# cyoq/onitama-alphazero

Hardware: AMD Instinct MI355X
Metric: MCTS node-expansions/sec/GPU @400 sims; self-play games/sec at 1/2/4/8 GPU (higher is better)
Workload: dtype fp32 (fp16x3 split)

## Files before the change

include/onitama_az.h:

```cpp
#ifndef ONITAMA_AZ_H
#define ONITAMA_AZ_H

#include <stddef.h>
#include <stdint.h>

#ifdef __cplusplus
extern "C" {
#endif

#define OAZ_ABI_VERSION 5

enum { OAZ_RED = 0, OAZ_BLUE = 1 };
enum { OAZ_PAWN = 0, OAZ_KING = 1 };
enum {
    OAZ_CAPTURE = 0,
    OAZ_RED_WIN = 1,
    OAZ_BLUE_WIN = 2,
    OAZ_IN_PROGRESS = 3
};
enum { OAZ_NUM_CARDS = 16, OAZ_MAX_MOVES = 40 };

enum {
    OAZ_OK = 0,
    OAZ_ERR_ARG = -1,
// ... 138 lines not shown
int oaz_set_search_time(oaz_engine* eng, int64_t search_time_ns);
int oaz_last_sims(oaz_engine* eng, int* sims);
int oaz_search_playouts(oaz_engine* eng, int* out, int G);
int oaz_load_weights(oaz_engine* eng, const float* blob, size_t n);

size_t oaz_weight_tensor_count(int blocks);
int oaz_weight_tensor_info(int blocks, size_t i, char* name, size_t name_cap, size_t* numel);
int oaz_weights_from_named(int blocks, const char* const* names, const float* const* data, const size_t* sizes,
                           size_t n, float* out, size_t out_n);
int oaz_load_weights_named(oaz_engine* eng, const char* const* names, const float* const* data,
                           const size_t* sizes, size_t n);
int oaz_ot_read(const char* path, float* out, size_t cap, size_t* n_out, int* blocks_out);
int oaz_load_ot(oaz_engine* eng, const char* path);
int oaz_ot_write(const char* path, const float* blob, size_t n, int blocks);
int oaz_checkpoint_path(const char* folder, int64_t iteration, int is_best, const char* stamp, char* out,
                        size_t cap);
int oaz_sync(oaz_engine* eng);
int oaz_set_timing(oaz_engine* eng, int enable);
int oaz_kernel_times_get(oaz_engine* eng, oaz_kernel_times* out);
int oaz_kernel_times_reset(oaz_engine* eng);

int oaz_nn_forward(oaz_engine* eng, const oaz_state* s, int B, float* policy, float* value);
int oaz_nn_fallbacks(oaz_engine* eng, uint64_t* tiles);

int oaz_search(oaz_engine* eng, const oaz_state* roots, int G, oaz_move* out_move,
               float* out_pi, float* out_root_value, oaz_search_stats* stats);
int oaz_tree_dump(oaz_engine* eng, int game, oaz_node* out, int cap, int* n_nodes);

int oaz_selfplay_reset(oaz_engine* eng);
int oaz_selfplay_step(oaz_engine* eng, int moves);
int oaz_selfplay_stats_get(oaz_engine* eng, oaz_selfplay_stats* out);
int oaz_samples_fetch(oaz_engine* eng, oaz_sample* out, size_t cap, size_t* n_out);
int oaz_samples_export_device(oaz_engine* eng, void* dev_dst, size_t cap_bytes, size_t* n_out);
int oaz_selfplay_run(oaz_engine* eng, int n_games, oaz_sample* out, size_t cap,
                     size_t* n_out, oaz_selfplay_stats* stats);

typedef struct oaz_comm oaz_comm;
typedef struct oaz_comm_id { char internal[128]; } oaz_comm_id;

int oaz_comm_unique_id(oaz_comm_id* out);
oaz_comm* oaz_comm_init(const oaz_comm_id* id, int rank, int world, int device);
void oaz_comm_destroy(oaz_comm* comm);
int oaz_allgather_samples(oaz_engine* eng, oaz_comm* comm, oaz_sample* dev_out, size_t cap, size_t* n_total,
                          uint64_t* counts_out);
int oaz_comm_allreduce_sum_f32(oaz_comm* comm, float* dev, size_t n, void* stream);
int oaz_comm_broadcast(oaz_comm* comm, void* dev, size_t bytes, int root, void* stream);
// ... 186 lines not shown
```

onitama-alphazero_amd/csrc/oaz_engine.cpp:

```cpp
#include <hip/hip_runtime.h>

#include <math.h>
#include <stddef.h>
#include <time.h>
#include <stdarg.h>
#include <stdio.h>
#include <stdlib.h>
#include <string.h>

#include <mutex>
#include <string>
#include <algorithm>
#include <vector>

#include "../../include/onitama_az.h"
#include "oaz_device.h"
#include "oaz_host.h"
#include "oaz_kernels.h"
#include "oaz_pack.h"
#include "oaz_weights_layout.h"

using namespace oaz;

static_assert(offsetof(oaz_config, search_time_ns) == 104 && sizeof(oaz_config) == 120, "oaz_config layout (ABI 4)");
// ... 658 lines not shown
extern "C" int oaz_nn_fallbacks(oaz_engine* e, uint64_t* tiles) {
    if (!e || !tiles) return oaz_set_err(OAZ_ERR_ARG, "nn_fallbacks: null");
    OAZ_ON_DEVICE(e->device);
    unsigned long long n = 0;
    HIP_TRY(hipMemcpyAsync(&n, e->nn_fallback, sizeof(n), hipMemcpyDeviceToHost, e->stream));
    HIP_TRY(hipStreamSynchronize(e->stream));
    *tiles = (uint64_t)n;
    return 0;
}

extern "C" int oaz_nn_forward(oaz_engine* e, const oaz_state* s, int B, float* policy, float* value) {
    if (!e || !s || B < 0) return oaz_set_err(OAZ_ERR_ARG, "nn_forward: bad arguments");
    if ((uint32_t)B > e->G) return oaz_set_err(OAZ_ERR_CAPACITY, "nn_forward: B=%d > games=%u", B, e->G);
    if (B == 0) return 0;
    OAZ_ON_DEVICE(e->device);
    HIP_TRY(hipMemcpyAsync(e->s_roots, s, (size_t)B * sizeof(oaz_state), hipMemcpyHostToDevice, e->stream));
    if (int rc = evaluate(e, e->s_roots, (uint32_t)B, e->s_rootp, e->s_rootv)) return rc;
    if (policy) HIP_TRY(hipMemcpyAsync(policy, e->s_rootp, (size_t)B * 50 * 4, hipMemcpyDeviceToHost, e->stream));
    if (value) HIP_TRY(hipMemcpyAsync(value, e->s_rootv, (size_t)B * 4, hipMemcpyDeviceToHost, e->stream));
    HIP_TRY(hipStreamSynchronize(e->stream));
    return 0;
}

static bool compact_leaves(const oaz_engine* e, uint32_t G) {
    return e->cfg.compact == 1 || (e->cfg.compact == 2 && G >= 12u * 16u * (uint32_t)e->cus);
}

enum SearchPath { PATH_LAT, PATH_GRP, PATH_STEPS };
static SearchPath search_path(const oaz_engine* e, uint32_t G, bool noise) {
    const bool one_launch = e->cfg.step_kernels == 0 && !compact_leaves(e, G) &&
                            (e->cfg.evaluator == OAZ_EVAL_HASH || e->cfg.precision == OAZ_FP32_SPLIT16) &&
                            tree_seg_kernels();
    if (!one_launch) return PATH_STEPS;
    if (!noise && G <= (uint32_t)e->cus) return PATH_LAT;
    return (G + 15) / 16 <= (uint32_t)e->cus ? PATH_GRP : PATH_STEPS;
}

static uint32_t noise_chunk_for(const oaz_engine* e) {
    if (search_path(e, e->G, true) != PATH_GRP) return kNoiseChunk;
    return std::max(kNoiseChunk, std::min((uint32_t)e->sims_cap, 512u));
}

constexpr uint32_t kAutoParts = 2048;
static int game_parts(const oaz_engine* e, uint32_t G) {
    int p = e->cfg.parts ? e->cfg.parts : (G >= kAutoParts ? 2 : 1);
    while (p > 1 && (uint32_t)(p - 1) * ((G + (uint32_t)p - 1) / (uint32_t)p) >= G) p /= 2;
// ... 475 lines not shown
```

onitama-alphazero_amd/csrc/oaz_nn.hip:

```cpp
#include <hip/hip_runtime.h>

#include <utility>

#include "oaz_device.h"
#include "oaz_kernels.h"

namespace oaz {

typedef float f32x4 __attribute__((ext_vector_type(4)));
typedef __bf16 bf16x8 __attribute__((ext_vector_type(8)));

namespace nn {
constexpr int kCh = 64;
constexpr int kSB = 16;
constexpr int kWaves = 8;
constexpr int kTPW = 13;
constexpr int kRS = 72;
constexpr int kScratch = 128;
constexpr int kLdsFloats = kSB * 25 * kRS + kWaves * kScratch;
}

struct TileSpan {
    int b0, end, cap;
};
__device__ __forceinline__ TileSpan tile_span(const TileMap& tm, int B) {
    if (!tm.bcnt) return TileSpan{(int)blockIdx.x * nn::kSB, B, B};
    const int b = (int)blockIdx.x % tm.nb, t = (int)blockIdx.x / tm.nb, base = b << kBucketShift;
    return TileSpan{base + t * nn::kSB, base + (int)tm.bcnt[b], tm.cap};
}

namespace x6 {
constexpr int kRowB = 384;
constexpr int kImageB = nn::kSB * 25 * kRowB;
constexpr int kLdsFloats = kImageB / 4 + nn::kWaves * nn::kScratch;
}

namespace h3 {
constexpr int kRowB = 128;
constexpr int kPlaneB = nn::kSB * 25 * kRowB;
constexpr int kImageB = 2 * kPlaneB;
constexpr int kLdsFloats = kImageB / 4 + nn::kWaves * nn::kScratch;
constexpr int kLutB = 256 * 16;
constexpr int kLutOff = kLdsFloats * 4;
}

__constant__ int8_t c_sq_order[25] = {0, 4, 20, 24, 1, 3, 21, 23, 6, 8, 12, 16, 18,
                                      2, 5, 10, 15, 9, 14, 19, 22, 7, 11, 13, 17};

__device__ __forceinline__ int nbr_index(int sq, int t) {
    const int r = sq / 5 + t / 3 - 1, c = sq % 5 + t % 3 - 1;
    return (r >= 0 && r < 5 && c >= 0 && c < 5) ? r * 5 + c : 25;
}

__device__ __forceinline__ int mover_info(const oaz_state st) {
    const int blue = st.to_move & 1;
    const int c0 = (blue ? st.cards[2] : st.cards[0]) & 15, c1 = (blue ? st.cards[3] : st.cards[1]) & 15;
    return c0 | (c1 << 4) | (blue << 8);
// ... 452 lines not shown
            B.nstep = -1;
            for (int i = 0; i < m; ++i) {
                B.j[i] = L.j[q + i];
                B.nb[i] = L.nb[q + i];
            }
            q += m;
            P.b[P.nbat++] = B;
        }
    }
    int next = -1;
    for (int k = P.nbat - 1; k >= 0; --k)
        if (P.b[k].first) {
            P.b[k].nstep = next;
            next = P.b[k].t * 2 + P.b[k].m;
        }
    return P;
}
template <int GRP, int KH>
struct ConvPlanOf {
    static constexpr ConvPlan P = conv_plan(GRP, KH);
};

struct X6Cfg {
    static constexpr int WAVES = 8, KH = OAZ_H3_KH, NS = 15, GRP0 = 3, GRP1 = 4;
};
template <int BF_, int DBG_ = 0>
struct H3Cfg {
    static constexpr int kSplit = BF_ ? kH1Split : kH3Split;
    static constexpr int WAVES = 8, KH = OAZ_H3_KH, NS = kSplit > 12 ? kSplit : 25 - kSplit, GRP0 = BF_ ? 9 : 7,
                         GRP1 = BF_ ? 10 : 8, BF = BF_, DBG = DBG_;
};

template <int GRP, int KH, int K, int N>
__device__ __forceinline__ void x6_load(bf16x8 (&a)[N], const char* img, const int (&ab)[2][3], int piece) {
    constexpr ConvBatch B = ConvPlanOf<GRP, KH>::P.b[K];
#pragma unroll
    for (int q = 0; q < N; ++q)
        if (q < B.n) {
            const int off = B.nb[q] * (nn::kSB * x6::kRowB) + piece * 128;
            a[q] = *reinterpret_cast<const bf16x8*>(img + ab[B.m][off >> 16] + (off & 0xffff));
        }
}

template <int GRP, int KH, int K, int NS, int N>
__device__ __forceinline__ void x6_mfma(f32x4 (&acc)[NS], const bf16x8 (&a)[N], const bf16x8& bv) {
    constexpr ConvBatch B = ConvPlanOf<GRP, KH>::P.b[K];
#pragma unroll
    for (int q = 0; q < N; ++q)
        if (q < B.n) acc[B.j[q]] = __builtin_amdgcn_mfma_f32_16x16x32_bf16(a[q], bv, acc[B.j[q]], 0, 0, 0);
}

struct FragW {
    __amdgpu_buffer_rsrc_t r;
    int voff;
};
__device__ __forceinline__ FragW frag_w(const float* p, size_t floats, int lane, int nt) {
    FragW w;
    w.r = __builtin_amdgcn_make_buffer_rsrc((void*)p, (short)0, (int)(floats * 4), 0x00020000);
    w.voff = (nt * 64 + lane) * 16;
    return w;
}
__device__ __forceinline__ bf16x8 x6_ldb(const FragW& w, int entry) {
    return __builtin_bit_cast(bf16x8, __builtin_amdgcn_raw_buffer_load_b128(w.r, w.voff, entry * 64 * 16, 0));
}

template <class C, int GRP, int K>
__device__ __forceinline__ void x6_step_b(const FragW& W, bf16x8 (&b)[3], bf16x8 (&bn)[3]) {
    constexpr ConvBatch B = ConvPlanOf<GRP, C::KH>::P.b[K];
    if constexpr (B.first && K > 0) {
#pragma unroll
        for (int pc = 0; pc < 3; ++pc) b[pc] = bn[pc];
    }
    if constexpr (B.first && B.nstep >= 0) {
#pragma unroll
        for (int pc = 0; pc < 3; ++pc) bn[pc] = x6_ldb(W, (B.nstep * 3 + pc) * 4);
    }
}

template <class C, int GRP, int K>
__device__ __forceinline__ void conv_x6_batch(f32x4 (&acc)[C::NS], const char* img, const FragW& W,
                                              bf16x8 (&b)[3], bf16x8 (&bn)[3], bf16x8 (&X)[C::KH],
                                              bf16x8 (&Y)[C::KH], const int (&ab)[2][3]) {
    constexpr int KH = C::KH, NS = C::NS;
    x6_step_b<C, GRP, K>(W, b, bn);
    x6_load<GRP, KH, K>(Y, img, ab, 0);
    x6_mfma<GRP, KH, K, NS>(acc, X, b[0]);
    x6_mfma<GRP, KH, K, NS>(acc, X, b[1]);
    x6_load<GRP, KH, K>(X, img, ab, 2);
    x6_mfma<GRP, KH, K, NS>(acc, Y, b[0]);
    x6_mfma<GRP, KH, K, NS>(acc, Y, b[1]);
    x6_mfma<GRP, KH, K, NS>(acc, Y, b[2]);
    if constexpr (K + 1 < ConvPlanOf<GRP, KH>::P.nbat) x6_load<GRP, KH, K + 1>(Y, img, ab, 1);
    x6_mfma<GRP, KH, K, NS>(acc, X, b[0]);
    __builtin_amdgcn_sched_barrier(0);
}

template <class C, int GRP, int... K>
__device__ __forceinline__ void conv_x6_run(f32x4 (&acc)[C::NS], const char* img, const FragW& W, const int (&lo)[2],
                                            std::integer_sequence<int, K...>) {
    int ab[2][3];
#pragma unroll
    for (int m = 0; m < 2; ++m)
#pragma unroll
        for (int sg = 0; sg < 3; ++sg) ab[m][sg] = lo[m] + sg * 65536;
    bf16x8 b[3], bn[3];
#pragma unroll
    for (int pc = 0; pc < 3; ++pc) b[pc] = x6_ldb(W, pc * 4);
    bf16x8 X[C::KH], Y[C::KH];
    x6_load<GRP, C::KH, 0>(X, img, ab, 1);
    ((K % 2 == 0 ? conv_x6_batch<C, GRP, K>(acc, img, W, b, bn, X, Y, ab)
                 : conv_x6_batch<C, GRP, K>(acc, img, W, b, bn, Y, X, ab)),
     ...);
}

template <class C, int GRP>
__device__ __forceinline__ void epilogue_x6_pack(const f32x4 (&acc)[C::NS], uint32_t (&pk)[C::NS][2][3],
                                                 const float* bias, f32x4 (&skip)[C::NS], int co, bool add,
                                                 bool keep) {
    const float bb = bias[co];
    const bool odd = co & 1;
    const float addf = add ? 1.0f : 0.0f;
    const uint32_t sel = odd ? 0x03020706u : 0x07060302u;
#pragma unroll
    for (int j = 0; j < grp_n(GRP); ++j) {
        float v[4];
#pragma unroll
        for (int r = 0; r < 4; ++r) {
            v[r] = __builtin_fmaf(skip[j][r], addf, acc[j][r] + bb);
            v[r] = v[r] > 0.0f ? v[r] : 0.0f;
            if (keep) skip[j][r] = v[r];
        }
#pragma unroll
        for (int k = 0; k < 2; ++k) {
            const float keep_ = odd ? v[2 * k + 1] : v[2 * k];
            const float send = odd ? v[2 * k] : v[2 * k + 1];
            const float got = __int_as_float(
                __builtin_amdgcn_update_dpp(0, __float_as_int(send), 0xB1, 0xF, 0xF, false));
            const uint32_t ka = __float_as_uint(keep_), ga = __float_as_uint(got);
            const float kr = keep_ - __uint_as_float(ka & 0xffff0000u), gr = got - __uint_as_float(ga & 0xffff0000u);
            const uint32_t kb = __float_as_uint(kr), gb = __float_as_uint(gr);
            const float kl = kr - __uint_as_float(kb & 0xffff0000u), gl = gr - __uint_as_float(gb & 0xffff0000u);
            pk[j][k][0] = __builtin_amdgcn_perm(ga, ka, sel);
            pk[j][k][1] = __builtin_amdgcn_perm(gb, kb, sel);
            pk[j][k][2] = __builtin_amdgcn_perm(__float_as_uint(gl), __float_as_uint(kl), sel);
        }
    }
}
template <class C, int GRP>
__device__ __forceinline__ void epilogue_x6_store(const uint32_t (&pk)[C::NS][2][3], char* img, const int (&eo)[2]) {
#pragma unroll
    for (int j = 0; j < grp_n(GRP); ++j)
#pragma unroll
        for (int k = 0; k < 2; ++k) {
            uint32_t* d = reinterpret_cast<uint32_t*>(img + grp_sq(GRP, j) * (nn::kSB * x6::kRowB) + eo[k]);
            d[0] = pk[j][k][0];
            d[32] = pk[j][k][1];
            d[64] = pk[j][k][2];
        }
}
template <class C, int GRP>
__device__ __forceinline__ void epilogue_x6(const f32x4 (&acc)[C::NS], char* img, const float* bias,
                                            f32x4 (&skip)[C::NS], const int (&eo)[2], int co, bool add, bool keep) {
    uint32_t pk[C::NS][2][3];
    epilogue_x6_pack<C, GRP>(acc, pk, bias, skip, co, add, keep);
    epilogue_x6_store<C, GRP>(pk, img, eo);
}

template <int GRP>
struct L1Regs {
    float w[9];
};
template <int GRP>
__device__ __forceinline__ void first_layer_x6_fetch(L1Regs<GRP>& R, const float* W, int lane, int nt) {
#pragma unroll
    for (int t = 0; t < 9; ++t) R.w[t] = W[(t * 4 + nt) * 64 + lane];
}
template <class C, int GRP>
__device__ __forceinline__ void first_layer_x6(f32x4 (&acc)[C::NS], const L1Regs<GRP>& R, const float* table,
                                               uint32_t bb, int cinfo, int lane, int nt) {
    const int kq = lane >> 4, co = nt * 16 + (lane & 15);
    constexpr int kBatch = 5;
    float tb[kBatch][5];
    auto fetch = [&](int j0) {
#pragma unroll
        for (int q = 0; q < kBatch; ++q)
            if (j0 + q < grp_n(GRP)) {
                const float* ts = table + (size_t)grp_sq(GRP, j0 + q) * 17 * nn::kCh + co;
#pragma unroll
// ... 17 lines not shown
        }
    const int c0 = cinfo & 15, c1 = (cinfo >> 4) & 15, blue = (cinfo >> 8) & 1;
    float a[5];
#pragma unroll
    for (int st = 0; st < 5; ++st) {
        const int k = 4 * st + kq;
        a[st] = k < 16 ? ((k == c0 || k == c1) ? 1.0f : 0.0f) : (k == 16 ? (float)blue : 0.0f);
    }
#pragma unroll
    for (int j0 = 0; j0 < grp_n(GRP); j0 += kBatch) {
#pragma unroll
        for (int st = 0; st < 5; ++st)
#pragma unroll
            for (int q = 0; q < kBatch; ++q)
                if (j0 + q < grp_n(GRP))
                    acc[j0 + q] = __builtin_amdgcn_mfma_f32_16x16x4f32(a[st], tb[q][st], acc[j0 + q], 0, 0, 0);
        if (j0 + kBatch < grp_n(GRP)) fetch(j0 + kBatch);
    }
}

template <class C, int GRP>
__device__ __forceinline__ void nn_x6_body(const oaz_state* __restrict__ states, const TileSpan sp,
                                           const float* __restrict__ blob, int blocks, float* __restrict__ policy,
                                           float* __restrict__ value, float* lds) {
    const int B = sp.end;
    constexpr int NS = C::NS;
    char* img = reinterpret_cast<char*>(lds);
    const int tid = threadIdx.x, wave = tid >> 6, lane = tid & 63;
    const int nt = wave & 3;
    const int b0 = sp.b0;
    int* pinfo = reinterpret_cast<int*>(lds + x6::kImageB / 4);
    const int co = nt * 16 + (lane & 15);
    const int i = lane & 15, kq = lane >> 4;
    int eo[2];
#pragma unroll
    for (int k = 0; k < 2; ++k) eo[k] = x6::elem_off(kq * 4 + 2 * k + (co & 1), co & ~1);
    const int lo[2] = {x6::chunk_off(i, 0, kq), x6::chunk_off(i, 0, 4 + kq)};

    f32x4 acc[NS];
    f32x4 skip[NS];
    {
        L1Regs<GRP> l1;
        first_layer_x6_fetch<GRP>(l1, blob + nnl::kL1B, lane, nt);
        const int b = min(b0 + i, sp.cap - 1);
        const uint32_t* w = reinterpret_cast<const uint32_t*>(&states[b]);
        const uint32_t bb = kq == 0 ? w[2] : kq == 1 ? w[0] : kq == 2 ? w[3] : w[1];
        if (tid < nn::kSB) pinfo[tid] = mover_info(states[b]);
        if (b0 >= B) return;
        __syncthreads();
#pragma unroll
        for (int j = 0; j < NS; ++j) acc[j] = skip[j] = f32x4{};
        first_layer_x6<C, GRP>(acc, l1, blob + nnl::kL1Table, bb, pinfo[i], lane, nt);
        epilogue_x6<C, GRP>(acc, img, blob + nnl::kL1Bias, skip, eo, co, false, true);
        __syncthreads();
    }
    const float* p = OAZ_NN_CONVS_AT(blob);
    for (int c = 0; c < 2 * blocks; ++c) {
#pragma unroll
        for (int j = 0; j < NS; ++j) acc[j] = f32x4{};
        conv_x6_run<C, GRP>(acc, img, frag_w(p, nnl::kConvW<OAZ_FP32_SPLIT>, lane, nt), lo,
                            std::make_integer_sequence<int, ConvPlanOf<GRP, C::KH>::P.nbat>{});
        p += nnl::kConvW<OAZ_FP32_SPLIT>;
        uint32_t pk[NS][2][3];
        epilogue_x6_pack<C, GRP>(acc, pk, p, skip, co, c & 1, c & 1);
        __syncthreads();
        epilogue_x6_store<C, GRP>(pk, img, eo);
        p += nnl::kConvTail<OAZ_FP32_SPLIT>;
        __syncthreads();
    }
    {
        const bf16x8* HB = reinterpret_cast<const bf16x8*>(p + nnl::kHeadB);
        bf16x8 hb[2][3];
#pragma unroll
        for (int m = 0; m < 2; ++m)
#pragma unroll
            for (int pc = 0; pc < 3; ++pc) hb[m][pc] = HB[(m * 3 + pc) * 64 + lane];
        constexpr int kSqPerWave = (25 + C::WAVES - 1) / C::WAVES;
        f32x4 hacc[kSqPerWave];
#pragma unroll
        for (int q = 0; q < kSqPerWave; ++q) {
            hacc[q] = f32x4{};
            const int sq = wave + q * C::WAVES;
            if (sq < 25) {
#pragma unroll
                for (int m = 0; m < 2; ++m) {
                    const char* a = img + sq * (nn::kSB * x6::kRowB) + lo[m];
                    const bf16x8 ah = *reinterpret_cast<const bf16x8*>(a);
                    const bf16x8 am = *reinterpret_cast<const bf16x8*>(a + 128);
                    const bf16x8 al = *reinterpret_cast<const bf16x8*>(a + 256);
                    hacc[q] = __builtin_amdgcn_mfma_f32_16x16x32_bf16(am, hb[m][0], hacc[q], 0, 0, 0);
                    hacc[q] = __builtin_amdgcn_mfma_f32_16x16x32_bf16(am, hb[m][1], hacc[q], 0, 0, 0);
                    hacc[q] = __builtin_amdgcn_mfma_f32_16x16x32_bf16(ah, hb[m][0], hacc[q], 0, 0, 0);
                    hacc[q] = __builtin_amdgcn_mfma_f32_16x16x32_bf16(ah, hb[m][1], hacc[q], 0, 0, 0);
                    hacc[q] = __builtin_amdgcn_mfma_f32_16x16x32_bf16(ah, hb[m][2], hacc[q], 0, 0, 0);
                    hacc[q] = __builtin_amdgcn_mfma_f32_16x16x32_bf16(al, hb[m][0], hacc[q], 0, 0, 0);
                }
            }
        }
        __syncthreads();
        float* feat = reinterpret_cast<float*>(img);
        const float hbias = i == 0 ? p[nnl::kBv] : i == 1 ? p[nnl::kBp] : p[nnl::kBp + 1];
#pragma unroll
        for (int q = 0; q < kSqPerWave; ++q) {
            const int sq = wave + q * C::WAVES;
            if (sq < 25 && i < 3)
#pragma unroll
                for (int r = 0; r < 4; ++r) {
                    const float v = hacc[q][r] + hbias;
                    feat[(kq * 4 + r) * 80 + i * 25 + sq] = v > 0.0f ? v : 0.0f;
                }
        }
        __syncthreads();
        constexpr int NP = nn::kSB / C::WAVES;
        const float* fq[NP];
        int bq[NP];
#pragma unroll
        for (int q = 0; q < NP; ++q) {
            fq[q] = feat + (wave + q * C::WAVES) * 80;
            bq[q] = b0 + wave + q * C::WAVES;
        }
        heads_mlp<NP>(fq, bq, p, lane, B, policy, value);
    }
}

template <class C>
__global__ void __launch_bounds__(64 * C::WAVES) k_nn_x6(const oaz_state* __restrict__ states, int B,
                                                        const float* __restrict__ blob, int blocks,
                                                        float* __restrict__ policy, float* __restrict__ value,
                                                        TileMap tm) {
    __shared__ __attribute__((aligned(16))) float lds[x6::kLdsFloats];
    const TileSpan sp = tile_span(tm, B);
    if ((threadIdx.x >> 8) == 0) {
        __builtin_amdgcn_s_setprio(1);
        nn_x6_body<C, C::GRP0>(states, sp, blob, blocks, policy, value, lds);
    } else {
        nn_x6_body<C, C::GRP1>(states, sp, blob, blocks, policy, value, lds);
// ... 457 lines not shown
        __syncthreads();
        stamp(4);
    };
    for (int c = 0; c < blocks; ++c) {
        conv_one(std::integral_constant<int, 0>{}, true);
        conv_one(std::integral_constant<int, 1>{}, c + 1 < blocks);
    }
    h3_heads<C>(p, img, lo, wave, lane, b0, B, policy, value);
    if constexpr (C::DBG == 2) {
        stamp(5);
        __syncthreads();
        float v = 0.0f;
#pragma unroll
        for (int k = 0; k < 8; ++k) v = lane == k ? (float)ph[k] : v;
        if (lane < 8 && b0 + nn::kSB <= B) policy[(size_t)b0 * 50 + wave * 8 + lane] = v;
    }
    if constexpr (C::BF) return false;
    return h3_overflowed(hmax);
}

template <class C>
struct H3Fallback {
    static constexpr bool kOn = !C::BF && C::DBG == 0;
    using X = X6Cfg;
    static constexpr int kBase = h3::kLdsFloats + h3::kLutB / 4;
    static constexpr int kLds = kOn && x6::kLdsFloats > kBase ? x6::kLdsFloats : kBase;
};

template <class X, int GRP>
__device__ __noinline__ void nn_h3_fallback(const oaz_state* __restrict__ states, const TileSpan sp,
                                            const float* __restrict__ xblob,
                                            int blocks, float* __restrict__ policy, float* __restrict__ value,
                                            float* lds) {
    nn_x6_body<X, GRP>(states, sp, xblob, blocks, policy, value, lds);
}

template <class C>
__global__ void __launch_bounds__(64 * C::WAVES) k_nn_h3(const oaz_state* __restrict__ states, int B,
                                                        const float* __restrict__ blob, int blocks,
                                                        float* __restrict__ policy, float* __restrict__ value,
                                                        const float* __restrict__ xblob,
                                                        unsigned long long* __restrict__ fallback, TileMap tm) {
    __shared__ __attribute__((aligned(16))) float lds[H3Fallback<C>::kLds];
    const uint64_t rt0 = C::DBG == 5 ? __builtin_amdgcn_s_memrealtime() : 0;
    const TileSpan sp = tile_span(tm, B);
    bool ovf;
    const bool g0 = (threadIdx.x >> 8) == 0;
    if (g0) {
        __builtin_amdgcn_s_setprio(1);
        ovf = nn_h3_body<C, C::GRP0>(states, sp, blob, blocks, policy, value, lds);
    } else {
        ovf = nn_h3_body<C, C::GRP1>(states, sp, blob, blocks, policy, value, lds);
    }
    if constexpr (H3Fallback<C>::kOn) {
        using X = typename H3Fallback<C>::X;
        if (__syncthreads_or(ovf)) {
            if (g0)
// ... 422 lines not shown
```

onitama-alphazero_amd/csrc/oaz_search_lat.hip:

```cpp
namespace oaz {

constexpr int kLatThreads = 512;

constexpr int kLatStateOff = h3s::kBytes;
constexpr int kLatVarsOff = kLatStateOff + 32;
constexpr int kLatPolOff = kLatVarsOff + 16;
constexpr int kLatStatOff = kLatPolOff + 52 * 4;
constexpr int kLatPathOff = kLatStatOff + GS_COUNT * 8;
constexpr int kLatPath = 2048;
constexpr int kLatSq = 2048;
constexpr int kLatLds = H3Fallback<H3Cfg<0>>::kLds * 4;
struct LatLayout {
    int root, sq, cache;
    uint32_t nsq, ncached;
};
__device__ __forceinline__ LatLayout lat_layout(uint32_t pathcap, bool path_lds, int sims, uint32_t cap) {
    LatLayout l;
    l.root = kLatPathOff + (path_lds ? (int)((pathcap * 4 + 15) & ~15u) : 0);
    l.sq = l.root + 32;
    l.nsq = (uint32_t)sims + 1 < (uint32_t)kLatSq ? (uint32_t)sims + 1 : (uint32_t)kLatSq;
    l.cache = (l.sq + (int)l.nsq * 8 + 31) & ~31;
    const uint32_t fit = (uint32_t)((kLatLds - l.cache) / (int)sizeof(oaz_node));
    l.ncached = fit < cap ? fit : cap;
    return l;
}

__device__ __noinline__ void lat_backup(const TreeView& t, const oaz_state* roots, const uint8_t* active,
                                        const float* policy, const float* value, uint32_t gs, float* sp,
                                        const NodesCached& na) {
    expand_backup_seg_body(t, roots, active, policy, value, gs, sp, na);
    __builtin_amdgcn_fence(__ATOMIC_RELEASE, "workgroup");
    __builtin_amdgcn_fence(__ATOMIC_ACQUIRE, "workgroup");
}
template <int DBG = 0>
// ... 115 lines not shown
        if (out) {
            *tg.n_nodes = *tl.n_nodes;
            *tg.leaf = *tl.leaf;
            *tg.depth = *tl.depth;
            *tg.leaf_state = *tl.leaf_state;
        } else {
            *tl.n_nodes = *tg.n_nodes;
            *tl.leaf = *tg.leaf;
            *tl.depth = *tg.depth;
            *tl.leaf_state = *tg.leaf_state;
        }
    }
}

template <int DBG = 0>
__global__ void __launch_bounds__(kLatThreads) k_search_lat(TreeView t, const oaz_state* __restrict__ roots,
                                                            const uint8_t* __restrict__ active, SearchParams prm,
                                                            int sims, int hash_eval, const float* __restrict__ blob,
                                                            int blocks, const float* __restrict__ xblob,
                                                            unsigned long long* __restrict__ fallback, float* policy,
                                                            float* value, const uint64_t* __restrict__ deadline,
                                                            uint32_t* __restrict__ sims_run) {
    using C = H3Cfg<0>;
    __shared__ __attribute__((aligned(16))) float lds[H3Fallback<C>::kLds];
    static_assert(kLatPathOff + kLatPath * 4 + 32 + kLatSq * 8 + 64 * (int)sizeof(oaz_node) <= kLatLds,
                  "k_search_lat LDS");
    const uint32_t g = blockIdx.x;
    if (g >= t.G || (active && active[g] != 1)) return;
    const int wave = (int)(threadIdx.x >> 6), lane = (int)(threadIdx.x & 63);
    const bool walker = wave == 4;
    char* const lb = reinterpret_cast<char*>(lds);
    TreeView tg = t;
    tg.nodes = t.nodes + (size_t)g * t.cap;
    tg.n_nodes = t.n_nodes + g;
    tg.path = t.path + (size_t)g * t.pathcap;
    tg.depth = t.depth + g;
    tg.leaf = t.leaf + g;
    tg.leaf_state = t.leaf_state + g;
    tg.stats = t.stats + (size_t)g * GS_COUNT;
    tg.need = nullptr;
    tg.slot = nullptr;
    tg.G = 1;
    const bool path_lds = t.pathcap <= (uint32_t)kLatPath;
    TreeView tl = tg;
    tl.leaf_state = reinterpret_cast<oaz_state*>(lb + kLatStateOff);
    tl.leaf = reinterpret_cast<uint32_t*>(lb + kLatVarsOff);
    tl.depth = tl.leaf + 1;
// ... 276 lines not shown
```

onitama-alphazero_amd/onitama_az/_abi.py:

```python
from __future__ import annotations

import ctypes as C
import os
from pathlib import Path

import numpy as np

LIB_NAME = "libonitama_az.so"
LIB_PATH = Path(__file__).resolve().parent / LIB_NAME

RED, BLUE = 0, 1
PAWN, KING = 0, 1
CAPTURE, RED_WIN, BLUE_WIN, IN_PROGRESS = 0, 1, 2, 3
EVAL_NN, EVAL_HASH = 0, 1
FP32, BF16, FP32_SPLIT, FP32_SPLIT16 = 0, 1, 2, 3
ERR_ARG = -1
ERR_RANGE = -7
ERR_CAPACITY = -4
ERR_COMM = -8
ABI_VERSION = 5
MAX_MOVES = 40


class OazError(RuntimeError):
# ... 278 lines not shown
    "oaz_encode": (C.c_int, [_VOIDP, C.c_int, _VOIDP]),
    "oaz_create": (_VOIDP, [_P(oaz_config), C.c_int]),
    "oaz_destroy": (None, [_VOIDP]),
    "oaz_get_config": (C.c_int, [_VOIDP, _P(oaz_config)]),
    "oaz_set_search_params": (C.c_int, [_VOIDP, C.c_int, C.c_double, C.c_int]),
    "oaz_set_search_time": (C.c_int, [_VOIDP, C.c_int64]),
    "oaz_last_sims": (C.c_int, [_VOIDP, _P(C.c_int)]),
    "oaz_search_playouts": (C.c_int, [_VOIDP, _VOIDP, C.c_int]),
    "oaz_load_weights": (C.c_int, [_VOIDP, _VOIDP, C.c_size_t]),
    "oaz_weight_tensor_count": (C.c_size_t, [C.c_int]),
    "oaz_weight_tensor_info": (C.c_int, [C.c_int, C.c_size_t, C.c_char_p, C.c_size_t, _P(C.c_size_t)]),
    "oaz_weights_from_named": (C.c_int, [C.c_int, _VOIDP, _VOIDP, _VOIDP, C.c_size_t, _VOIDP, C.c_size_t]),
    "oaz_load_weights_named": (C.c_int, [_VOIDP, _VOIDP, _VOIDP, _VOIDP, C.c_size_t]),
    "oaz_ot_read": (C.c_int, [C.c_char_p, _VOIDP, C.c_size_t, _P(C.c_size_t), _P(C.c_int)]),
    "oaz_load_ot": (C.c_int, [_VOIDP, C.c_char_p]),
    "oaz_ot_write": (C.c_int, [C.c_char_p, _VOIDP, C.c_size_t, C.c_int]),
    "oaz_checkpoint_path": (C.c_int, [C.c_char_p, C.c_int64, C.c_int, C.c_char_p, C.c_char_p, C.c_size_t]),
    "oaz_sync": (C.c_int, [_VOIDP]),
    "oaz_set_timing": (C.c_int, [_VOIDP, C.c_int]),
    "oaz_kernel_times_get": (C.c_int, [_VOIDP, _P(oaz_kernel_times)]),
    "oaz_kernel_times_reset": (C.c_int, [_VOIDP]),
    "oaz_nn_forward": (C.c_int, [_VOIDP, _VOIDP, C.c_int, _VOIDP, _VOIDP]),
    "oaz_nn_fallbacks": (C.c_int, [_VOIDP, _P(C.c_uint64)]),
    "oaz_search": (C.c_int, [_VOIDP, _VOIDP, C.c_int, _VOIDP, _VOIDP, _VOIDP, _P(oaz_search_stats)]),
    "oaz_tree_dump": (C.c_int, [_VOIDP, C.c_int, _VOIDP, C.c_int, _P(C.c_int)]),
    "oaz_selfplay_reset": (C.c_int, [_VOIDP]),
    "oaz_selfplay_step": (C.c_int, [_VOIDP, C.c_int]),
    "oaz_selfplay_stats_get": (C.c_int, [_VOIDP, _P(oaz_selfplay_stats)]),
    "oaz_samples_fetch": (C.c_int, [_VOIDP, _VOIDP, C.c_size_t, _P(C.c_size_t)]),
    "oaz_samples_export_device": (C.c_int, [_VOIDP, _VOIDP, C.c_size_t, _P(C.c_size_t)]),
    "oaz_selfplay_run": (C.c_int, [_VOIDP, C.c_int, _VOIDP, C.c_size_t, _P(C.c_size_t), _P(oaz_selfplay_stats)]),
    "oaz_comm_unique_id": (C.c_int, [_P(oaz_comm_id)]),
    "oaz_comm_init": (_VOIDP, [_P(oaz_comm_id), C.c_int, C.c_int, C.c_int]),
    "oaz_comm_destroy": (None, [_VOIDP]),
    "oaz_allgather_samples": (C.c_int, [_VOIDP, _VOIDP, _VOIDP, C.c_size_t, _P(C.c_size_t), _VOIDP]),
    "oaz_comm_allreduce_sum_f32": (C.c_int, [_VOIDP, _VOIDP, C.c_size_t, _VOIDP]),
    "oaz_comm_broadcast": (C.c_int, [_VOIDP, _VOIDP, C.c_size_t, C.c_int, _VOIDP]),
    "oaz_comm_sync": (C.c_int, [_VOIDP]),
    "oaz_comm_stats_get": (C.c_int, [_VOIDP, _P(oaz_comm_stats)]),
    "oaz_pure_mcts_config_default": (None, [_P(oaz_pure_mcts_config)]),
    "oaz_pure_mcts_tree_capacity": (C.c_size_t, [_P(oaz_pure_mcts_config)]),
    "oaz_pure_mcts_search": (C.c_int, [_VOIDP, C.c_int, _P(oaz_pure_mcts_config), _VOIDP, _VOIDP,
                                       _P(oaz_pure_mcts_stats), _VOIDP, C.c_size_t]),
    "oaz_pure_mcts_release_workspace": (C.c_int, [C.c_int]),
    "oaz_alphabeta_config_default": (None, [_P(oaz_alphabeta_config)]),
    "oaz_alphabeta_evaluate": (C.c_int, [_VOIDP, _VOIDP, C.c_int, _VOIDP]),
# ... 16 lines not shown
    "oaz_train_config_default": (None, [_P(oaz_train_config)]),
    "oaz_trainer_create": (_VOIDP, [_P(oaz_train_config), C.c_int]),
    "oaz_trainer_destroy": (None, [_VOIDP]),
    "oaz_trainer_set_stream": (C.c_int, [_VOIDP, _VOIDP]),
    "oaz_trainer_set_weights": (C.c_int, [_VOIDP, _VOIDP, C.c_size_t]),
    "oaz_trainer_get_weights": (C.c_int, [_VOIDP, _VOIDP, C.c_size_t]),
    "oaz_trainer_save_ot": (C.c_int, [_VOIDP, C.c_char_p]),
    "oaz_trainer_load_samples": (C.c_int, [_VOIDP, _VOIDP, C.c_size_t]),
    "oaz_trainer_bind_device_samples": (C.c_int, [_VOIDP, _VOIDP, C.c_size_t]),
    "oaz_trainer_set_batches": (C.c_int, [_VOIDP, _VOIDP, C.c_int, C.c_int]),
    "oaz_trainer_backward": (C.c_int, [_VOIDP, C.c_int]),
    "oaz_trainer_grads": (C.c_int, [_VOIDP, _P(C.c_void_p), _P(C.c_size_t)]),
    "oaz_trainer_get_grads": (C.c_int, [_VOIDP, _VOIDP, C.c_size_t]),
    "oaz_trainer_apply": (C.c_int, [_VOIDP, C.c_float]),
    "oaz_trainer_bn_stats_count": (C.c_size_t, [C.c_int]),
    "oaz_trainer_bn_stats_pack": (C.c_int, [_VOIDP, _VOIDP]),
    "oaz_trainer_bn_stats_unpack": (C.c_int, [_VOIDP, _VOIDP, C.c_float]),
    "oaz_trainer_train": (C.c_int, [_VOIDP, C.c_int, C.c_int]),
    "oaz_trainer_losses": (C.c_int, [_VOIDP, _P(C.c_double * 3)]),
    "oaz_trainer_sync": (C.c_int, [_VOIDP]),
}

EXPORTED_SYMBOLS = tuple(_PROTOS)

_lib = None


def load(path: str | os.PathLike | None = None) -> C.CDLL:
    global _lib
    if _lib is not None and path is None:
        return _lib
    p = Path(path) if path else Path(os.environ["OAZ_LIB"]) if os.environ.get("OAZ_LIB") else LIB_PATH
    if not p.exists():
        raise OazError(f"{p} not found: build it with `python -c 'import __graft_entry__ as g; g.build()'`")
    lib = C.CDLL(str(p), mode=C.RTLD_GLOBAL)
    for name, (res, args) in _PROTOS.items():
        fn = getattr(lib, name)
        fn.restype = res
        fn.argtypes = args
    if lib.oaz_abi_version() != ABI_VERSION:
        raise OazError("ABI version mismatch")
    if path is None:
        _lib = lib
    return lib


def check(rc: int) -> None:
    if rc < 0:
        msg = load().oaz_last_error()
        raise OazError(f"C ABI error {rc}: {msg.decode() if msg else ''}")


def ptr(a: np.ndarray) -> C.c_void_p:
    assert a.flags["C_CONTIGUOUS"]
    return C.c_void_p(a.ctypes.data)


def device_count() -> int:
    n = C.c_int(0)
    load().oaz_device_count(C.byref(n))
# ... 8 lines not shown
```

onitama-alphazero_amd/onitama_az/engine.py:

```python
from __future__ import annotations

import ctypes as C
from dataclasses import dataclass
from typing import Optional, Tuple

import numpy as np

from . import _abi


@dataclass
class SearchResult:
    moves: np.ndarray
    pi: np.ndarray
    root_value: Optional[np.ndarray]
    stats: _abi.oaz_search_stats


class Engine:

    def __init__(self, config: Optional[_abi.oaz_config] = None, device: int = 0, **overrides):
        lib = _abi.load()
        cfg = config if config is not None else _abi.default_config()
        for k, v in overrides.items():
# ... 42 lines not shown
        _abi.check(self._lib.oaz_set_search_time(self._h, int(round(float(seconds) * 1e9))))

    def last_sims(self) -> int:
        n = C.c_int(0)
        _abi.check(self._lib.oaz_last_sims(self._h, C.byref(n)))
        return int(n.value)

    def search_playouts(self, games: int) -> np.ndarray:
        out = np.zeros(int(games), dtype=np.int32)
        _abi.check(self._lib.oaz_search_playouts(self._h, _abi.ptr(out), int(games)))
        return out

    def sync(self) -> None:
        _abi.check(self._lib.oaz_sync(self._h))

    def nn_forward(self, states: np.ndarray) -> Tuple[np.ndarray, np.ndarray]:
        states = np.ascontiguousarray(states, dtype=_abi.STATE_DTYPE)
        B = len(states)
        pol = np.zeros((B, 2, 25), dtype=np.float32)
        val = np.zeros(B, dtype=np.float32)
        _abi.check(self._lib.oaz_nn_forward(self._h, _abi.ptr(states), B, _abi.ptr(pol), _abi.ptr(val)))
        return pol, val

    def nn_fallbacks(self) -> int:
        n = C.c_uint64(0)
        _abi.check(self._lib.oaz_nn_fallbacks(self._h, C.byref(n)))
        return int(n.value)

    def search(self, roots: np.ndarray, root_value: bool = False) -> SearchResult:
        roots = np.ascontiguousarray(roots, dtype=_abi.STATE_DTYPE)
        G = len(roots)
        moves = np.zeros(G, dtype=_abi.MOVE_DTYPE)
        pi = np.zeros((G, 2, 25), dtype=np.float32)
        rv = np.zeros(G, dtype=np.float32) if root_value else None
        st = _abi.oaz_search_stats()
        _abi.check(self._lib.oaz_search(self._h, _abi.ptr(roots), G, _abi.ptr(moves), _abi.ptr(pi),
                                        _abi.ptr(rv) if rv is not None else None, C.byref(st)))
        return SearchResult(moves, pi, rv, st)

    def tree(self, game: int) -> np.ndarray:
        n = C.c_int(0)
        _abi.check(self._lib.oaz_tree_dump(self._h, game, None, 0, C.byref(n)))
        out = np.zeros(n.value, dtype=_abi.NODE_DTYPE)
        _abi.check(self._lib.oaz_tree_dump(self._h, game, _abi.ptr(out), n.value, C.byref(n)))
        return out

# ... 40 lines not shown
```

Before: 51.60 million.

## Run the h3 fallback recompute in two half-tile passes within h3's LDS

The x6 fallback path inside the h3 network kernel now processes the 16-row tile in two 8-row passes, so its image fits in the h3 kernel's own LDS footprint. Previously the fallback's larger LDS need inflated the h3 kernel's and the latency search kernel's shared-memory allocation. The intent is to shrink per-block LDS and so raise occupancy for the common h3 path, at the cost of a slower fallback that now recomputes per half-tile. A tiled forward entry point is also added for testing the bucketed path.

```diff
diff --git a/include/onitama_az.h b/include/onitama_az.h
--- a/include/onitama_az.h
+++ b/include/onitama_az.h
@@ -184,6 +184,7 @@
 
 int oaz_nn_forward(oaz_engine* eng, const oaz_state* s, int B, float* policy, float* value);
 int oaz_nn_fallbacks(oaz_engine* eng, uint64_t* tiles);
+int oaz_nn_forward_tiled(oaz_engine* eng, const oaz_state* s, int B, int count, float* policy, float* value);
 
 int oaz_search(oaz_engine* eng, const oaz_state* roots, int G, oaz_move* out_move,
                float* out_pi, float* out_root_value, oaz_search_stats* stats);
diff --git a/onitama-alphazero_amd/csrc/oaz_engine.cpp b/onitama-alphazero_amd/csrc/oaz_engine.cpp
--- a/onitama-alphazero_amd/csrc/oaz_engine.cpp
+++ b/onitama-alphazero_amd/csrc/oaz_engine.cpp
@@ -704,6 +704,30 @@
     return 0;
 }
 
+extern "C" int oaz_nn_forward_tiled(oaz_engine* e, const oaz_state* s, int B, int count, float* policy, float* value) {
+    if (!e || !s || B < 0 || count > B) return oaz_set_err(OAZ_ERR_ARG, "nn_forward_tiled: bad arguments");
+    if ((uint32_t)B > e->G) return oaz_set_err(OAZ_ERR_CAPACITY, "nn_forward_tiled: B=%d > games=%u", B, e->G);
+    if (e->cfg.evaluator != OAZ_EVAL_NN) return oaz_set_err(OAZ_ERR_ARG, "nn_forward_tiled: the engine's evaluator is not the network");
+    if (count >= 0 && (uint32_t)B > kBucket) return oaz_set_err(OAZ_ERR_ARG, "nn_forward_tiled: one bucket holds %u rows", kBucket);
+    if (B == 0) return 0;
+    OAZ_ON_DEVICE(e->device);
+    const uint32_t cnt = count >= 0 ? (uint32_t)count : 0u;
+    HIP_TRY(hipMemcpyAsync(e->s_roots, s, (size_t)B * sizeof(oaz_state), hipMemcpyHostToDevice, e->stream));
+    const TileMap tm{e->bcnt, 1, B};
+    if (count >= 0) {
+        HIP_TRY(hipMemcpyAsync(e->bcnt, &cnt, sizeof(cnt), hipMemcpyHostToDevice, e->stream));
+        HIP_TRY(hipMemsetAsync(e->s_rootp, 0, (size_t)B * 50 * 4, e->stream));
+        HIP_TRY(hipMemsetAsync(e->s_rootv, 0, (size_t)B * 4, e->stream));
+    }
+    NNView w = nn_view(e, count >= 0 ? &tm : nullptr);
+    w.small_max = 0;
+    HIP_TRY(launch_nn_forward(w, e->s_roots, B, e->s_rootp, e->s_rootv, e->stream));
+    if (policy) HIP_TRY(hipMemcpyAsync(policy, e->s_rootp, (size_t)B * 50 * 4, hipMemcpyDeviceToHost, e->stream));
+    if (value) HIP_TRY(hipMemcpyAsync(value, e->s_rootv, (size_t)B * 4, hipMemcpyDeviceToHost, e->stream));
+    HIP_TRY(hipStreamSynchronize(e->stream));
+    return 0;
+}
+
 static bool compact_leaves(const oaz_engine* e, uint32_t G) {
     return e->cfg.compact == 1 || (e->cfg.compact == 2 && G >= 12u * 16u * (uint32_t)e->cus);
 }
diff --git a/onitama-alphazero_amd/csrc/oaz_nn.hip b/onitama-alphazero_amd/csrc/oaz_nn.hip
--- a/onitama-alphazero_amd/csrc/oaz_nn.hip
+++ b/onitama-alphazero_amd/csrc/oaz_nn.hip
@@ -33,6 +33,8 @@
 constexpr int kRowB = 384;
 constexpr int kImageB = nn::kSB * 25 * kRowB;
 constexpr int kLdsFloats = kImageB / 4 + nn::kWaves * nn::kScratch;
+constexpr int image_bytes(int rows) { return rows * 25 * kRowB; }
+constexpr int lds_floats(int rows) { return image_bytes(rows) / 4 + nn::kWaves * nn::kScratch; }
 }
 
 namespace h3 {
@@ -531,7 +533,10 @@
 };
 
 struct X6Cfg {
-    static constexpr int WAVES = 8, KH = OAZ_H3_KH, NS = 15, GRP0 = 3, GRP1 = 4;
+    static constexpr int WAVES = 8, KH = OAZ_H3_KH, NS = 15, GRP0 = 3, GRP1 = 4, ROWS = nn::kSB;
+};
+struct X6HalfCfg : X6Cfg {
+    static constexpr int ROWS = 8;
 };
 template <int BF_, int DBG_ = 0>
 struct H3Cfg {
@@ -540,13 +545,13 @@
                          GRP1 = BF_ ? 10 : 8, BF = BF_, DBG = DBG_;
 };
 
-template <int GRP, int KH, int K, int N>
+template <int ROWS, int GRP, int KH, int K, int N>
 __device__ __forceinline__ void x6_load(bf16x8 (&a)[N], const char* img, const int (&ab)[2][3], int piece) {
     constexpr ConvBatch B = ConvPlanOf<GRP, KH>::P.b[K];
 #pragma unroll
     for (int q = 0; q < N; ++q)
         if (q < B.n) {
-            const int off = B.nb[q] * (nn::kSB * x6::kRowB) + piece * 128;
+            const int off = B.nb[q] * (ROWS * x6::kRowB) + piece * 128;
             a[q] = *reinterpret_cast<const bf16x8*>(img + ab[B.m][off >> 16] + (off & 0xffff));
         }
 }
@@ -592,14 +597,14 @@
                                               bf16x8 (&Y)[C::KH], const int (&ab)[2][3]) {
     constexpr int KH = C::KH, NS = C::NS;
     x6_step_b<C, GRP, K>(W, b, bn);
-    x6_load<GRP, KH, K>(Y, img, ab, 0);
+    x6_load<C::ROWS, GRP, KH, K>(Y, img, ab, 0);
     x6_mfma<GRP, KH, K, NS>(acc, X, b[0]);
     x6_mfma<GRP, KH, K, NS>(acc, X, b[1]);
-    x6_load<GRP, KH, K>(X, img, ab, 2);
+    x6_load<C::ROWS, GRP, KH, K>(X, img, ab, 2);
     x6_mfma<GRP, KH, K, NS>(acc, Y, b[0]);
     x6_mfma<GRP, KH, K, NS>(acc, Y, b[1]);
     x6_mfma<GRP, KH, K, NS>(acc, Y, b[2]);
-    if constexpr (K + 1 < ConvPlanOf<GRP, KH>::P.nbat) x6_load<GRP, KH, K + 1>(Y, img, ab, 1);
+    if constexpr (K + 1 < ConvPlanOf<GRP, KH>::P.nbat) x6_load<C::ROWS, GRP, KH, K + 1>(Y, img, ab, 1);
     x6_mfma<GRP, KH, K, NS>(acc, X, b[0]);
     __builtin_amdgcn_sched_barrier(0);
 }
@@ -616,7 +621,7 @@
 #pragma unroll
     for (int pc = 0; pc < 3; ++pc) b[pc] = x6_ldb(W, pc * 4);
     bf16x8 X[C::KH], Y[C::KH];
-    x6_load<GRP, C::KH, 0>(X, img, ab, 1);
+    x6_load<C::ROWS, GRP, C::KH, 0>(X, img, ab, 1);
     ((K % 2 == 0 ? conv_x6_batch<C, GRP, K>(acc, img, W, b, bn, X, Y, ab)
                  : conv_x6_batch<C, GRP, K>(acc, img, W, b, bn, Y, X, ab)),
      ...);
@@ -656,12 +661,14 @@
     }
 }
 template <class C, int GRP>
-__device__ __forceinline__ void epilogue_x6_store(const uint32_t (&pk)[C::NS][2][3], char* img, const int (&eo)[2]) {
+__device__ __forceinline__ void epilogue_x6_store(const uint32_t (&pk)[C::NS][2][3], char* img, const int (&eo)[2],
+                                                  bool own) {
+    if (C::ROWS < nn::kSB && !own) return;
 #pragma unroll
     for (int j = 0; j < grp_n(GRP); ++j)
 #pragma unroll
         for (int k = 0; k < 2; ++k) {
-            uint32_t* d = reinterpret_cast<uint32_t*>(img + grp_sq(GRP, j) * (nn::kSB * x6::kRowB) + eo[k]);
+            uint32_t* d = reinterpret_cast<uint32_t*>(img + grp_sq(GRP, j) * (C::ROWS * x6::kRowB) + eo[k]);
             d[0] = pk[j][k][0];
             d[32] = pk[j][k][1];
             d[64] = pk[j][k][2];
@@ -669,10 +676,11 @@
 }
 template <class C, int GRP>
 __device__ __forceinline__ void epilogue_x6(const f32x4 (&acc)[C::NS], char* img, const float* bias,
-                                            f32x4 (&skip)[C::NS], const int (&eo)[2], int co, bool add, bool keep) {
+                                            f32x4 (&skip)[C::NS], const int (&eo)[2], bool own, int co, bool add,
+                                            bool keep) {
     uint32_t pk[C::NS][2][3];
     epilogue_x6_pack<C, GRP>(acc, pk, bias, skip, co, add, keep);
-    epilogue_x6_store<C, GRP>(pk, img, eo);
+    epilogue_x6_store<C, GRP>(pk, img, eo, own);
 }
 
 template <int GRP>
@@ -736,19 +744,20 @@
 template <class C, int GRP>
 __device__ __forceinline__ void nn_x6_body(const oaz_state* __restrict__ states, const TileSpan sp,
                                            const float* __restrict__ blob, int blocks, float* __restrict__ policy,
-                                           float* __restrict__ value, float* lds) {
+                                           float* __restrict__ value, float* lds, int pass = 0) {
     const int B = sp.end;
-    constexpr int NS = C::NS;
+    constexpr int NS = C::NS, ROWS = C::ROWS, kSqB = ROWS * x6::kRowB;
     char* img = reinterpret_cast<char*>(lds);
     const int tid = threadIdx.x, wave = tid >> 6, lane = tid & 63;
     const int nt = wave & 3;
-    const int b0 = sp.b0;
-    int* pinfo = reinterpret_cast<int*>(lds + x6::kImageB / 4);
+    const int b0 = sp.b0 + pass * ROWS;
+    int* pinfo = reinterpret_cast<int*>(lds + x6::image_bytes(ROWS) / 4);
     const int co = nt * 16 + (lane & 15);
-    const int i = lane & 15, kq = lane >> 4;
+    const int i = lane & (ROWS - 1), kq = lane >> 4;
+    const bool own = kq * 4 < ROWS;
     int eo[2];
 #pragma unroll
-    for (int k = 0; k < 2; ++k) eo[k] = x6::elem_off(kq * 4 + 2 * k + (co & 1), co & ~1);
+    for (int k = 0; k < 2; ++k) eo[k] = x6::elem_off((kq * 4 + 2 * k + (co & 1)) & (ROWS - 1), co & ~1);
     const int lo[2] = {x6::chunk_off(i, 0, kq), x6::chunk_off(i, 0, 4 + kq)};
 
     f32x4 acc[NS];
@@ -759,13 +768,13 @@
         const int b = min(b0 + i, sp.cap - 1);
         const uint32_t* w = reinterpret_cast<const uint32_t*>(&states[b]);
         const uint32_t bb = kq == 0 ? w[2] : kq == 1 ? w[0] : kq == 2 ? w[3] : w[1];
-        if (tid < nn::kSB) pinfo[tid] = mover_info(states[b]);
+        if (tid < ROWS) pinfo[tid] = mover_info(states[b]);
         if (b0 >= B) return;
         __syncthreads();
 #pragma unroll
         for (int j = 0; j < NS; ++j) acc[j] = skip[j] = f32x4{};
         first_layer_x6<C, GRP>(acc, l1, blob + nnl::kL1Table, bb, pinfo[i], lane, nt);
-        epilogue_x6<C, GRP>(acc, img, blob + nnl::kL1Bias, skip, eo, co, false, true);
+        epilogue_x6<C, GRP>(acc, img, blob + nnl::kL1Bias, skip, eo, own, co, false, true);
         __syncthreads();
     }
     const float* p = OAZ_NN_CONVS_AT(blob);
@@ -778,7 +787,7 @@
         uint32_t pk[NS][2][3];
         epilogue_x6_pack<C, GRP>(acc, pk, p, skip, co, c & 1, c & 1);
         __syncthreads();
-        epilogue_x6_store<C, GRP>(pk, img, eo);
+        epilogue_x6_store<C, GRP>(pk, img, eo, own);
         p += nnl::kConvTail<OAZ_FP32_SPLIT>;
         __syncthreads();
     }
@@ -798,7 +807,7 @@
             if (sq < 25) {
 #pragma unroll
                 for (int m = 0; m < 2; ++m) {
-                    const char* a = img + sq * (nn::kSB * x6::kRowB) + lo[m];
+                    const char* a = img + sq * kSqB + lo[m];
                     const bf16x8 ah = *reinterpret_cast<const bf16x8*>(a);
                     const bf16x8 am = *reinterpret_cast<const bf16x8*>(a + 128);
                     const bf16x8 al = *reinterpret_cast<const bf16x8*>(a + 256);
@@ -813,19 +822,20 @@
         }
         __syncthreads();
         float* feat = reinterpret_cast<float*>(img);
-        const float hbias = i == 0 ? p[nnl::kBv] : i == 1 ? p[nnl::kBp] : p[nnl::kBp + 1];
+        const int hc = lane & 15;
+        const float hbias = hc == 0 ? p[nnl::kBv] : hc == 1 ? p[nnl::kBp] : p[nnl::kBp + 1];
 #pragma unroll
         for (int q = 0; q < kSqPerWave; ++q) {
             const int sq = wave + q * C::WAVES;
-            if (sq < 25 && i < 3)
+            if (sq < 25 && hc < 3 && own)
 #pragma unroll
                 for (int r = 0; r < 4; ++r) {
                     const float v = hacc[q][r] + hbias;
-                    feat[(kq * 4 + r) * 80 + i * 25 + sq] = v > 0.0f ? v : 0.0f;
+                    feat[(kq * 4 + r) * 80 + hc * 25 + sq] = v > 0.0f ? v : 0.0f;
                 }
         }
         __syncthreads();
-        constexpr int NP = nn::kSB / C::WAVES;
+        constexpr int NP = ROWS / C::WAVES;
         const float* fq[NP];
         int bq[NP];
 #pragma unroll
@@ -1329,17 +1339,26 @@
 template <class C>
 struct H3Fallback {
     static constexpr bool kOn = !C::BF && C::DBG == 0;
-    using X = X6Cfg;
+    using X = X6HalfCfg;
     static constexpr int kBase = h3::kLdsFloats + h3::kLutB / 4;
-    static constexpr int kLds = kOn && x6::kLdsFloats > kBase ? x6::kLdsFloats : kBase;
+    static constexpr int kLds = kBase;
+    static_assert(x6::lds_floats(X::ROWS) <= kLds, "the recompute runs in k_nn_h3's own LDS");
 };
 
+template <class X, int GRP>
+__device__ __noinline__ void nn_h3_fallback_pass(const oaz_state* __restrict__ states, const TileSpan sp,
+                                                 const float* __restrict__ xblob,
+                                                 int blocks, float* __restrict__ policy, float* __restrict__ value,
+                                                 float* lds, int pass) {
+    nn_x6_body<X, GRP>(states, sp, xblob, blocks, policy, value, lds, pass);
+}
 template <class X, int GRP>
 __device__ __noinline__ void nn_h3_fallback(const oaz_state* __restrict__ states, const TileSpan sp,
-                                            const float* __restrict__ xblob,
-                                            int blocks, float* __restrict__ policy, float* __restrict__ value,
-                                            float* lds) {
-    nn_x6_body<X, GRP>(states, sp, xblob, blocks, policy, value, lds);
+                                               const float* __restrict__ xblob, int blocks,
+                                               float* __restrict__ policy, float* __restrict__ value, float* lds) {
+#pragma nounroll
+    for (int pass = 0; pass < nn::kSB / X::ROWS; ++pass)
+        nn_h3_fallback_pass<X, GRP>(states, sp, xblob, blocks, policy, value, lds, pass);
 }
 
 template <class C>
diff --git a/onitama-alphazero_amd/csrc/oaz_search_lat.hip b/onitama-alphazero_amd/csrc/oaz_search_lat.hip
--- a/onitama-alphazero_amd/csrc/oaz_search_lat.hip
+++ b/onitama-alphazero_amd/csrc/oaz_search_lat.hip
@@ -9,7 +9,8 @@
 constexpr int kLatPathOff = kLatStatOff + GS_COUNT * 8;
 constexpr int kLatPath = 2048;
 constexpr int kLatSq = 2048;
-constexpr int kLatLds = H3Fallback<H3Cfg<0>>::kLds * 4;
+constexpr int kLatLds = x6::kLdsFloats * 4;
+static_assert(kLatLds >= H3Fallback<H3Cfg<0>>::kLds * 4, "k_search_lat holds the network's LDS");
 struct LatLayout {
     int root, sq, cache;
     uint32_t nsq, ncached;
@@ -171,7 +172,7 @@
                                                             float* value, const uint64_t* __restrict__ deadline,
                                                             uint32_t* __restrict__ sims_run) {
     using C = H3Cfg<0>;
-    __shared__ __attribute__((aligned(16))) float lds[H3Fallback<C>::kLds];
+    __shared__ __attribute__((aligned(16))) float lds[kLatLds / 4];
     static_assert(kLatPathOff + kLatPath * 4 + 32 + kLatSq * 8 + 64 * (int)sizeof(oaz_node) <= kLatLds,
                   "k_search_lat LDS");
     const uint32_t g = blockIdx.x;
diff --git a/onitama-alphazero_amd/onitama_az/_abi.py b/onitama-alphazero_amd/onitama_az/_abi.py
--- a/onitama-alphazero_amd/onitama_az/_abi.py
+++ b/onitama-alphazero_amd/onitama_az/_abi.py
@@ -324,6 +324,7 @@
     "oaz_kernel_times_reset": (C.c_int, [_VOIDP]),
     "oaz_nn_forward": (C.c_int, [_VOIDP, _VOIDP, C.c_int, _VOIDP, _VOIDP]),
     "oaz_nn_fallbacks": (C.c_int, [_VOIDP, _P(C.c_uint64)]),
+    "oaz_nn_forward_tiled": (C.c_int, [_VOIDP, _VOIDP, C.c_int, C.c_int, _VOIDP, _VOIDP]),
     "oaz_search": (C.c_int, [_VOIDP, _VOIDP, C.c_int, _VOIDP, _VOIDP, _VOIDP, _P(oaz_search_stats)]),
     "oaz_tree_dump": (C.c_int, [_VOIDP, C.c_int, _VOIDP, C.c_int, _P(C.c_int)]),
     "oaz_selfplay_reset": (C.c_int, [_VOIDP]),
@@ -386,6 +387,7 @@
 }
 
 EXPORTED_SYMBOLS = tuple(_PROTOS)
+_ADDED_IN_ABI_5 = ("oaz_nn_forward_tiled",)
 
 _lib = None
 
@@ -399,7 +401,11 @@
         raise OazError(f"{p} not found: build it with `python -c 'import __graft_entry__ as g; g.build()'`")
     lib = C.CDLL(str(p), mode=C.RTLD_GLOBAL)
     for name, (res, args) in _PROTOS.items():
-        fn = getattr(lib, name)
+        fn = getattr(lib, name, None)
+        if fn is None and path is None and os.environ.get("OAZ_LIB") and name in _ADDED_IN_ABI_5:
+            continue
+        if fn is None:
+            raise OazError(f"{p}: no symbol {name}")
         fn.restype = res
         fn.argtypes = args
     if lib.oaz_abi_version() != ABI_VERSION:
diff --git a/onitama-alphazero_amd/onitama_az/engine.py b/onitama-alphazero_amd/onitama_az/engine.py
--- a/onitama-alphazero_amd/onitama_az/engine.py
+++ b/onitama-alphazero_amd/onitama_az/engine.py
@@ -88,6 +88,14 @@
         _abi.check(self._lib.oaz_nn_forward(self._h, _abi.ptr(states), B, _abi.ptr(pol), _abi.ptr(val)))
         return pol, val
 
+    def nn_forward_tiled(self, states: np.ndarray, count: int = -1) -> Tuple[np.ndarray, np.ndarray]:
+        states = np.ascontiguousarray(states, dtype=_abi.STATE_DTYPE)
+        B = len(states)
+        pol = np.zeros((B, 2, 25), dtype=np.float32)
+        val = np.zeros(B, dtype=np.float32)
+        _abi.check(self._lib.oaz_nn_forward_tiled(self._h, _abi.ptr(states), B, count, _abi.ptr(pol), _abi.ptr(val)))
+        return pol, val
+
     def nn_fallbacks(self) -> int:
         n = C.c_uint64(0)
         _abi.check(self._lib.oaz_nn_fallbacks(self._h, C.byref(n)))
```

Result: no change. 51.81 million, median of 6 (+0.4%).
